# SumitTarafder/Figbird

Measured on AMD Instinct MI355X. Metric: gaps/sec (+ filled-bases/sec), synthetic 1e5-gap set recipe, jump-library fill pass, higher is better.
Workload: dtype f64

## Files before the change

### figbird_amd/api.py

```python
from __future__ import annotations

import ctypes as C
import os
from dataclasses import dataclass
from typing import List, Optional

import numpy as np

from . import build as _build

c_double_p = C.POINTER(C.c_double)
c_i32_p = C.POINTER(C.c_int32)
c_i64_p = C.POINTER(C.c_int64)
c_u8_p = C.POINTER(C.c_uint8)


class FigModel(C.Structure):
    _fields_ = [
        ("max_read_length", C.c_int32), ("error_pos_dist", c_double_p), ("in_pos_dist", c_double_p),
        ("del_pos_dist", c_double_p), ("error_type_probs", C.c_double * 25),
        ("insert_len_dist_smoothed", c_double_p), ("max_insert_size", C.c_int32),
        ("insert_threshold_min", C.c_int32), ("insert_threshold_max", C.c_int32), ("gap_prob_cutoff", C.c_int32),
        ("partial_flag", C.c_int32), ("unmapped_flag", C.c_int32), ("script_itr", C.c_int32),
        ("max_distance", C.c_int32), ("read_length", C.c_int32), ("neg_overlap", C.c_int32),
# ... 17 lines not shown
class FigGapResults(C.Structure):
    _fields_ = [
        ("filled_len", c_i32_p), ("gaptofill", c_i32_p), ("str_off", c_i64_p), ("str", C.c_char_p),
        ("str_capacity", C.c_int64),
        ("dbg_max_cand", C.c_int32), ("dbg_n_cand", c_i32_p), ("dbg_cand_i", c_i32_p), ("dbg_cand_lik", c_double_p),
        ("dbg_n_place", c_i32_p),
        ("draw_pos", c_i32_p), ("draw_isz", c_i32_p), ("draw_len", c_i32_p),
        ("dbg_plane_cols", C.c_int32), ("dbg_plane_reads", C.c_int32), ("dbg_counts", c_double_p), ("dbg_read_maxlv", c_double_p),
    ]


class FigStats(C.Structure):
    _fields_ = [("kernel_ms", C.c_double), ("h2d_ms", C.c_double), ("d2h_ms", C.c_double),
                ("packed_bytes", C.c_int64), ("place_calls", C.c_int64), ("alg_flops", C.c_double),
                ("n_launches", C.c_int32), ("pad0", C.c_int32), ("spec_flops", C.c_double),
                ("mle_alg_flops", C.c_double), ("mle_exec_flops", C.c_double)]


EXPORTS = ["fig_version", "fig_strerror", "fig_ctx_create", "fig_ctx_destroy", "fig_ctx_set_model",
           "fig_results_capacity", "fig_batch_upload", "fig_fill_resident", "fig_batch_free", "fig_fill_gaps",
           "fig_get_stats", "fig_batch_probe_reach", "fig_batch_set_ot_preset"]

_lib = None
_host = None


def load_library(path: Optional[str] = None) -> C.CDLL:
    global _lib
    if _lib is not None and path is None:
        return _lib
    p = path or _build.LIB
# ... 321 lines not shown
```

### figbird_amd/csrc/fig_abi.hip

```cpp
#include <hip/hip_runtime.h>

#include <algorithm>
#include <cstdio>
#include <cstdlib>
#include <cstring>
#include <new>
#include <vector>
#include <chrono>
#include <thread>
#include <mutex>

#include "../../include/figbird_hip.h"
#include "fig_engine.h"
#include "fig_pack.h"
#include "fig_abi_host.h"

#ifdef FIG_PROF
#define FIG_PROF_BEGIN() const unsigned long long _k0 = __builtin_readcyclecounter()
#define FIG_PROF_FLUSH() do { if (E.lane == 0) { atomicAdd(&B.counters[30], E.wait_cycles); atomicAdd(&B.counters[31], (unsigned long long)__builtin_readcyclecounter() - _k0); \
    for (int i = 0; i < 22; i++) if (E.prof[i]) atomicAdd(&B.counters[8 + i], E.prof[i]); \
    for (int i = 22; i < 40; i++) if (E.prof[i]) atomicAdd(&B.counters[32 + (i - 22)], E.prof[i]); } } while (0)
#else
#define FIG_PROF_BEGIN() ((void)0)
#define FIG_PROF_FLUSH() ((void)0)
// ... 194 lines not shown
    DevBuf d_model_tabs;
    fig_model hm;
    bool have_batch = false;
    FigDevBatch db;
    std::vector<FigDevGap> h_gaps;
    std::vector<int32_t> h_order;
    struct Cls { FigLaunchClass c; int blocks; int capacity; };
    std::vector<Cls> classes;
    std::vector<DevBuf> bufs;
    int64_t n_gaps = 0, n_ureads = 0, n_preads = 0, str_total = 0;
    std::vector<int64_t> h_str_off;
    int nslots = 32;
    std::vector<FigLane> lanes;
    fig_stats stats;
    int sh_on = FIG_SH_SC;
    std::vector<uint8_t> h_ot;
    uint8_t *d_ot = nullptr;
};

static int dev_alloc(fig_ctx *ctx, size_t bytes, void **out) {
    DevBuf b;
    if (bytes == 0) bytes = 8;
    hipError_t e = hipMalloc(&b.p, bytes);
    if (e != hipSuccess) { ctx->last_hip = (int)e; return FIG_ENOMEM; }
    b.n = bytes;
    ctx->bufs.push_back(b);
    *out = b.p;
    return FIG_OK;
}

// ... 22 lines not shown
    int n = 0;
    if (hipGetDeviceCount(&n) != hipSuccess || n <= 0) return FIG_ENODEV;
    if (device_ordinal < 0 || device_ordinal >= n) return FIG_ENODEV;
    if (hipSetDevice(device_ordinal) != hipSuccess) return FIG_ENODEV;
    hipDeviceProp_t prop;
    if (hipGetDeviceProperties(&prop, device_ordinal) != hipSuccess) return FIG_ENODEV;
    fig_ctx *ctx = new (std::nothrow) fig_ctx();
    if (!ctx) return FIG_ENOMEM;
    ctx->device = device_ordinal;
    ctx->n_cu = prop.multiProcessorCount > 0 ? prop.multiProcessorCount : 256;
    if (hipStreamCreate(&ctx->stream) != hipSuccess || hipEventCreate(&ctx->ev0) != hipSuccess || hipEventCreate(&ctx->ev1) != hipSuccess) {
        delete ctx;
        return FIG_EHIP;
    }
    memset(&ctx->stats, 0, sizeof(ctx->stats));
    ctx->sh_on = fig_knobs_from_env(0).sh_on;
    *out = ctx;
    return FIG_OK;
}

static void free_batch(fig_ctx *ctx) {
    for (auto &b : ctx->bufs) if (b.p) hipFree(b.p);
    ctx->bufs.clear();
    ctx->d_ot = nullptr;
    ctx->have_batch = false;
    ctx->classes.clear();
    for (auto &l : ctx->lanes) { if (l.stream) hipStreamDestroy(l.stream); if (l.done) hipEventDestroy(l.done); if (l.h_ctl) hipHostFree(l.h_ctl); if (l.h_items) hipHostFree(l.h_items); if (l.h_entries) hipHostFree(l.h_entries); }
    ctx->lanes.clear();
}

extern "C" void fig_batch_free(fig_ctx *ctx) {
// ... 60 lines not shown

static hipError_t launch_any(fig_ctx *ctx, const fig_ctx::Cls &c, const FigDevBatch &db, hipStream_t stream, FigKind kind, int blocks, const void *list, int n, int qsel = 0) {
    if (c.c.tiles > 0) return launch_kind<true, 512>(ctx, c, db, stream, kind, blocks, list, n, qsel);
    if (c.c.lds_tab) return c.c.nt == 256 ? launch_kind<true, 256>(ctx, c, db, stream, kind, blocks, list, n, qsel) : launch_kind<true, 512>(ctx, c, db, stream, kind, blocks, list, n, qsel);
    return launch_kind<false, 512>(ctx, c, db, stream, kind, blocks, list, n, qsel);
}

extern "C" int fig_batch_upload(fig_ctx *ctx, const fig_gap_batch *b) {
    if (!ctx || !b) return FIG_EINVAL;
    if (!ctx->have_model) return FIG_EINVAL;
    hipSetDevice(ctx->device);
    free_batch(ctx);
    const fig_model *m = &ctx->hm;
    hipEventRecord(ctx->ev0, ctx->stream);
    FigPacked K;
    int prc = fig_pack(m, b, sizeof(FigState), K);
    if (prc) return prc;
    int64_t ng = K.n_gaps;
    ctx->h_gaps = K.gaps; ctx->h_order = K.order; ctx->h_str_off = K.str_off;
    ctx->str_total = K.str_total; ctx->n_gaps = ng;
    ctx->n_ureads = (int64_t)K.u_pos.size(); ctx->n_preads = (int64_t)K.p_pos.size();
    ctx->classes.clear();
    const bool log = fig_knobs_from_env(0).log;
    for (const FigLaunchClass &lc : K.classes) {
        fig_ctx::Cls c;
        c.c = lc;
        int per_cu = (int)std::max<size_t>(1, std::min<size_t>((160 * 1024) / std::max<size_t>(lc.lds, 1), (size_t)(2048 / lc.nt)));
        per_cu = std::min(per_cu, 8);
        c.capacity = ctx->n_cu * per_cu;
        c.blocks = std::min<int>(lc.q_end - lc.q_begin, c.capacity);
// ... 265 lines not shown
    ctx->stats.d2h_ms = ms;
#ifdef FIG_PROF
    { const char *nm[14] = {"A.wait", "B.wait", "-", "M.finish", "PR.pre", "PR.estep", "PR.mid", "PR.mle", "PR.post", "A.chain", "A.logexp", "A.work", "B.work", "M.chains"};
      for (int i = 0; i < 14; i++) fprintf(stderr, "[figprof] %-9s %8.1f Gcycles = %5.1f %% of wave-cycles\n", nm[i], cnt[8 + i] / 1e9, cnt[31] ? 100.0 * cnt[8 + i] / cnt[31] : 0.0);
      { const char *mn[4] = {"M.setup", "M.hint", "M.rounds", "M.surv"};
        for (int i = 0; i < 4; i++) fprintf(stderr, "[figprof] %-9s %8.1f Gcycles = %5.1f %% of wave-cycles\n", mn[i], cnt[22 + i] / 1e9, cnt[31] ? 100.0 * cnt[22 + i] / cnt[31] : 0.0); }
      fprintf(stderr, "[figprof] raw slots:"); for (int i = 0; i < 22; i++) fprintf(stderr, " %d:%.1f", i, cnt[8 + i] / 1e9); for (int i = 22; i < 40; i++) fprintf(stderr, " %d:%.1f", i, cnt[32 + i - 22] / 1e9); fprintf(stderr, "\n");
      fprintf(stderr, "[figprof] barrier wait %.3f of %.3f wave-Gcycles = %.1f %%\n", cnt[30] / 1e9, cnt[31] / 1e9, cnt[31] ? 100.0 * cnt[30] / cnt[31] : 0.0); }
#endif
    if (knobs.log) fprintf(stderr, "[figsched] useful flops %.4g, speculative evaluations executed %.4g (%.1f %% discarded)\n", (double)cnt[1], (double)cnt[2], cnt[2] ? 100.0 * (1.0 - ((double)cnt[1] / (double)cnt[2])) : 0.0);
    ctx->stats.place_calls = (int64_t)cnt[0];
    ctx->stats.alg_flops = (double)cnt[1];
    ctx->stats.spec_flops = (double)cnt[2];
    ctx->stats.mle_alg_flops = (double)cnt[3];
    ctx->stats.mle_exec_flops = (double)cnt[4];
    return fig_compact_results(ng, hstr.data(), ctx->h_str_off.data(), out);
}

extern "C" int fig_fill_gaps(fig_ctx *ctx, const fig_gap_batch *batch, fig_gap_results *out) { return fig_fill_gaps_once(ctx, batch, out); }

extern "C" int fig_get_stats(const fig_ctx *ctx, fig_stats *out) {
    if (!ctx || !out) return FIG_EINVAL;
    *out = ctx->stats;
    return FIG_OK;
}
```

### figbird_amd/csrc/fig_abi_host.h

```cpp
#ifndef FIG_ABI_HOST_H
#define FIG_ABI_HOST_H
#include <algorithm>
#include <cmath>
#include <cstdlib>
#include <cstring>
#include <vector>
#include "../../include/figbird_hip.h"
#include "fig_types.h"
#include "fig_gaprules.h"

static inline const char *fig_strerror_text(int code) {
    switch (code) {
        case FIG_OK: return "ok";
        case FIG_EINVAL: return "invalid argument";
        case FIG_ENODEV: return "no usable HIP device (libfighip has no CPU path)";
        case FIG_ENOMEM: return "out of memory";
        case FIG_EHIP: return "HIP runtime error";
        case FIG_ENOSPC: return "result string buffer too small";
        case FIG_EUNSUP: return "input outside the supported envelope";
        default: return "unknown error";
    }
}

static inline int fig_model_check(const fig_model *m) {
// ... 89 lines not shown
static int fig_fill_gaps_once(fig_ctx *ctx, const fig_gap_batch *batch, fig_gap_results *out) {
    int rc = fig_batch_upload(ctx, batch);
    if (rc) return rc;
    rc = fig_fill_resident(ctx, out);
    fig_batch_free(ctx);
    return rc;
}

struct FigKnobs {
    bool seq;
    bool lanes_serial;
    bool log;
    int minc;
    double ipw;
    int sh_on;
};

static FigKnobs fig_knobs_from_env(int unmapped) {
    FigKnobs k;
    const char *sched = getenv("FIG_SCHED"), *ser = getenv("FIG_LANES"), *mc = getenv("FIG_MIN_CHUNK"), *ipw = getenv("FIG_ITEMS_PER_WG");
    const char *ev = getenv("FIG_ESTEP"), *sc = getenv("FIG_SH_CHUNKS");
    k.seq = sched && strcmp(sched, "seq") == 0;
    k.lanes_serial = ser && strcmp(ser, "serial") == 0;
    k.log = getenv("FIG_SCHED_LOG") != nullptr;
    k.minc = mc ? std::max(1, atoi(mc)) : 16;
    k.ipw = ipw ? std::max(1.0, atof(ipw)) : (unmapped ? 12.0 : 6.0);
    k.sh_on = (ev && !strcmp(ev, "pair")) ? 0 : (sc ? std::max(1, std::min(FIG_SH_SC, atoi(sc))) : FIG_SH_SC);
    return k;
}

struct FigRound { std::vector<int> items, entries; int chunk = 0, n_active = 0; };

static void fig_plan_round(const std::vector<int> &ids, const int32_t *ctl, int capacity, int nsplit, int slots_cap, int minc, double ipw_base,
                           int &n_active_max, FigRound &R) {
    std::vector<int> &items = R.items, &entries = R.entries;
    items.clear(); entries.clear();
    R.chunk = 0; R.n_active = 0;
    for (int g : ids) if (ctl[(size_t)g * 4] == 1) R.n_active++;
    if (R.n_active == 0) return;
    long long rem_total = 0;
    for (int g : ids) if (ctl[(size_t)g * 4] == 1) rem_total += std::max(0, ctl[(size_t)g * 4 + 2] - ctl[(size_t)g * 4 + 1]);
    n_active_max = std::max(n_active_max, R.n_active);
// ... 21 lines not shown
```

### figbird_amd/csrc/fig_engine.h

```cpp
#ifndef FIG_ENGINE_H
#define FIG_ENGINE_H

#include "fig_types.h"

#ifdef FIG_EMU
#include <cmath>
#include <cstring>
#define FIG_D static inline
#define FIG_NOINLINE
#define FIG_HD static inline
#define FIG_SYNC() ((void)0)
FIG_D double fig_log10(double x) { return log10(x); }
FIG_D double fig_log(double x) { return log(x); }
FIG_D double fig_exp(double x) { return exp(x); }
FIG_D double fig_pow10(double x) { return pow(10, x); }
FIG_D int fig_atomic_add_i32(int *p, int v) { int o = *p; *p += v; return o; }
FIG_D void fig_atomic_max_i32(int *p, int v) { if (v > *p) *p = v; }
FIG_D int fig_atomic_fetch_add_i32(int *p, int v) { int o = *p; *p += v; return o; }
FIG_D void fig_atomic_min_i32(int *p, int v) { if (v < *p) *p = v; }
FIG_D void fig_atomic_or_i32(int *p, int v) { *p |= v; }
FIG_D void fig_atomic_add_u64(unsigned long long *p, unsigned long long v) { *p += v; }
FIG_D unsigned long long fig_shfl_down_u64(unsigned long long v, int off) { (void)v; (void)off; return 0; }
#else
#include <hip/hip_runtime.h>
// ... 81 lines not shown
    unsigned char gap_left[32], gap_right[32];
    unsigned char partial_left[100], partial_right[100];
    double FP[6][5], FQ[6][5];
    double red_v[16]; int red_i[16];
    double bc_d; int bc_i, bc_j;
    int ibuf[8];
    double lik;
    int ctl[8];
    int tm_lo[16], tm_hi[16], tm_len[16], tm_tis0[16], tm_dir[16];
    int tm_aux[16]; long long tm_woff[16];
    double wv_v[32]; int wv_o[32];
    short sh_lo[FIG_SH_SC * FIG_SH_C], sh_hi[FIG_SH_SC * FIG_SH_C];
    int sh_tis0[FIG_SH_SC * FIG_SH_C];
    unsigned sh_woff[FIG_SH_SC * FIG_SH_C];
    unsigned char sh_len[FIG_SH_SC * FIG_SH_C], sh_aux[FIG_SH_SC * FIG_SH_C];
    unsigned sh_irr[16], sh_pad;
    int mle_next, pad_mn;
    int fin_i[8];
    FigLoop L;
    unsigned long long flops_useful; int n_place, pad_np;
    int dbg_j, pad_dj;
};

struct FigTrip { int v[3]; };



struct FigScr {
    double *cnt;
    double *ncnt;
    double *tmp;
    int *pc;
    int *nci;
    unsigned char *accf;
    unsigned char *mdone;
    int *cov;
// ... 454 lines not shown
```

### figbird_amd/csrc/fig_engine_core.h

```cpp

struct FigWin { int lo, hi; int tis0; int dir; };

FIG_D FigWin fig_window_unmapped(const FigEng &E, int pos1, int len, int G, int gapoffset) {
    const FigDevModel &M = *E.M;
    long long gsl = E.g->gapStart;
    FigWin w;
    int lo = -(len - 1), hi = G - 1;
    if ((long long)pos1 < gsl) {
        w.tis0 = (int)(gsl - pos1 + len); w.dir = 1;
        int a = M.Tmin - w.tis0, b = M.Tmax - w.tis0;
        if (a > lo) lo = a;
        if (b < hi) hi = b;
    } else {
        int p = pos1 + gapoffset;
        w.tis0 = (int)(p - gsl + len); w.dir = -1;
        int a = w.tis0 - M.Tmax, b = w.tis0 - M.Tmin;
        if (a > lo) lo = a;
        if (b < hi) hi = b;
    }
    w.lo = lo; w.hi = hi;
    return w;
}

FIG_D FigWin fig_window_partial(const FigEng &E, int pos1, int ref_pos, int len, int G, int gapoffset, int shift_always) {
// ... 288 lines not shown
                        if (S.gap_right[s4n + j] == rc) match++;
                    }
                    if (remn - match <= 2) return s4n;
                }
                part_count++;
                if (part_count > FIG_READ_CAP) break;
            }
        }
    }
    return 0;
}

FIG_D int fig_initialize(FigEng &E, int gl, int negGapCheck) {
    FigState &S = *E.S;
    int cg = E.capG;
    if (E.tid == 0) { S.G = gl; fig_ise(E); S.region_perct = 0; }
    FIG_SYNC();
    int G = S.G;
    for (int x = E.tid; x < cg; x += E.nt) {
        if (x < G) { E.scr.cnt[x] = 0; E.scr.cnt[cg + x] = 0; E.scr.cnt[2 * cg + x] = 0; E.scr.cnt[3 * cg + x] = 0; E.scr.cnt[4 * cg + x] = 1;
                     for (int j = 0; j < 5; j++) E.scr.ncnt[j * cg + x] = 0; }
        for (int j = 0; j < 5; j++) E.scr.tmp[j * cg + x] = 0;
        E.scr.cov[x] = 0;
    }
    int nml = E.g->nU > E.g->nP ? E.g->nU : E.g->nP;
    for (int r = E.tid; r < nml; r += E.nt) E.scr.maxlv[r] = 0;
    for (int r = E.tid; r < E.g->nU; r += E.nt) { E.scr.hint[r] = FIG_NOPOS; E.scr.hint_e[r] = FIG_NOPOS; }
    FIG_SYNC();
    if (E.tid == 0) {
        int gfp = 0;
        if (S.side_limit > 0 && negGapCheck == 0) gfp = fig_find_contig_match(E);
// ... 949 lines not shown
```

### figbird_amd/csrc/fig_engine_sched.h

```cpp
#ifndef FIG_ENGINE_SCHED_H
#define FIG_ENGINE_SCHED_H

template <bool LDS>
FIG_D void fig_gap_begin(FigEng &E) {
    FigState &S = *E.S;
    const FigDevModel &M = *E.M;
    const FigDevGap &g = *E.g;
    int G0 = g.G0, nU = g.nU;
    if (E.tid == 0) {
        S.left = M.D; S.right = M.D; S.side_limit = 30; S.end_pos_max = 0;
        S.valid_count = S.invalid_count = 0;
        S.partial_read_count = M.partial_flag == 1 ? g.nP : 0;
        S.region_perct = 0; S.region_perct_max = 0;
        S.partial_read_len = M.partial_len;
        S.rep_flag = 0; S.one_side_repeat_flag = 0; S.large_gap_flag = g.lgf; S.comp_count = 0;
        S.left_max = 0; S.right_min = 0; S.discont_or_not = 0;
        S.psr_temp[0] = S.psr_temp[1] = S.psr_final[0] = S.psr_final[1] = -1;
        S.umaxleftf = S.umaxrightf = S.ucoverf = 0;
        S.num_itr = 0; S.overlap_threshold = (E.B->ot_preset && E.B->ot_preset[g.gapNo]) ? 5 : 0; S.gaptofill = 0;
        S.gl_len = S.gr_len = S.pl_len = S.pr_len = 0;
        S.cons_len = 1; E.scr.cons[0] = 4;
        E.scr.used_read_arr[0] = 0;
        S.best_len = S.cur_len = S.prev_len = S.orig_len = 0;
        S.flops_useful = 0; S.n_place = 0; S.dbg_j = -1; S.pad_dj = 0;
        fig_flank_tables(E);
        if (E.B->dbg_n_cand) E.B->dbg_n_cand[g.gapNo] = 0;
        if (E.B->draw_len) { E.B->draw_len[(long long)g.gapNo * 2] = -1; E.B->draw_len[(long long)g.gapNo * 2 + 1] = -1; }
    }
    for (int r = E.tid; r < nU; r += E.nt) {
        E.scr.saved[r] = 0; E.scr.mark[r] = 0; E.scr.org[r * 2] = -200; E.scr.org[r * 2 + 1] = 0;
        E.scr.frp[r * 2] = -200; E.scr.frp[r * 2 + 1] = 0;
        if (E.B->draw_pos) E.B->draw_pos[g.uBase + r] = (int)0x80000000;
    }
    for (int p = E.tid; p < g.nP; p += E.nt) {
        E.scr.ppos_org[p * 3] = 0; E.scr.ppos_org[p * 3 + 1] = -200; E.scr.ppos_org[p * 3 + 2] = 0;
        if (E.B->draw_pos) E.B->draw_pos[E.B->n_ureads + g.pBase + p] = (int)0x80000000;
    }
    FIG_SYNC();
    if (E.tid == 0) {
// ... 273 lines not shown
FIG_D unsigned char *fig_slot_mark(const FigPersist &P, int s, int capGg) { return fig_slot_cons(P, s) + 2 * fig_align8(capGg + 8); }

FIG_D void fig_state_save(FigEng &E, const FigPersist &P) {
    FIG_SYNC();
    const int n = (int)(sizeof(FigState) / 4);
    const int *src = (const int *)E.S; int *dst = (int *)P.state;
    for (int i = E.tid; i < n; i += E.nt) dst[i] = src[i];
    FIG_SYNC();
}
FIG_D void fig_state_load(FigEng &E, const FigPersist &P) {
    FIG_SYNC();
    const int n = (int)(sizeof(FigState) / 4);
    int *dst = (int *)E.S; const int *src = (const int *)P.state;
    for (int i = E.tid; i < n; i += E.nt) dst[i] = src[i];
    FIG_SYNC();
}

enum { FIG_BIND_SEQ = 0, FIG_BIND_EVAL = 1, FIG_BIND_REPLAY = 2 };
FIG_D void fig_bind(FigEng &E, const FigScr &work, const FigPersist &P, int mode, int slot, int capGg) {
    E.scr = work;
    E.scr.best = P.best; E.scr.orig = P.orig; E.scr.saved = P.saved;
    E.scr.repeatflag = P.repeatflag; E.scr.used_read_arr = P.used_read_arr; E.scr.lrmd = P.lrmd;
    E.scr.org = P.org; E.scr.ppos_org = P.ppos_org;
    if (mode == FIG_BIND_SEQ) { E.scr.prev = P.prev; }
    else {
        E.scr.cons = fig_slot_cons(P, slot); E.scr.mark = fig_slot_mark(P, slot, capGg);
        if (mode == FIG_BIND_EVAL) { E.scr.org = P.org_spec; E.scr.ppos_org = P.ppos_spec; }
    }
}

// ... 82 lines not shown
```

### figbird_amd/csrc/fig_engine_shared.h

```cpp
#ifndef FIG_ENGINE_SHARED_H
#define FIG_ENGINE_SHARED_H
#ifndef FIG_EMU
#define FIG_FI __device__ static __forceinline__

FIG_D unsigned fig_wave_max_u32(unsigned v) {
#define FIG_DPP_UMAX(ctrl, rmask) do { const unsigned y_ = (unsigned)__builtin_amdgcn_update_dpp(0, (int)v, ctrl, rmask, 0xf, false); v = y_ > v ? y_ : v; } while (0)
    FIG_DPP_UMAX(0x111, 0xf); FIG_DPP_UMAX(0x112, 0xf); FIG_DPP_UMAX(0x114, 0xf); FIG_DPP_UMAX(0x118, 0xf);
    FIG_DPP_UMAX(0x142, 0xa); FIG_DPP_UMAX(0x143, 0xc);
#undef FIG_DPP_UMAX
    return (unsigned)__builtin_amdgcn_readlane((int)v, 63);
}


template <int N>
FIG_FI void fig_weights_n(const double (&x)[N], double (&w)[N]) {
    double m[N], a[N], b[N], r[N], s[N], z[N], q[N], s_lo[N], t[N], lm_lo[N], ed[N], p_hi[N], p_lo[N], r_hi[N], sum[N], err[N], tl[N];
    int e[N];
#pragma unroll
    for (int i = 0; i < N; i++) { m[i] = __builtin_amdgcn_frexp_mant(x[i]); e[i] = __builtin_amdgcn_frexp_exp(x[i]); }
#pragma unroll
    for (int i = 0; i < N; i++) { const bool lowhalf = m[i] < 0.70710678118654752440; m[i] = lowhalf ? m[i] + m[i] : m[i]; e[i] = lowhalf ? e[i] - 1 : e[i]; }
#pragma unroll
    for (int i = 0; i < N; i++) { a[i] = m[i] - 1.0; b[i] = m[i] + 1.0; }
#pragma unroll
// ... 80 lines not shown
    double f[8], m1[8], m2[8];
#pragma unroll
    for (int b = 0; b < 4; b++) { m1[b] = ac[b].p * kc[0]; m1[4 + b] = ac[b].p * kc[2]; }
#pragma unroll
    for (int b = 0; b < 4; b++) { m2[b] = kc[1] * ac[b].q; m2[4 + b] = kc[3] * ac[b].q; }
#pragma unroll
    for (int i = 0; i < 8; i++) f[i] = m1[i] + m2[i];
    const double one = 1.0;
    if (NS == 32) { fig_sh_mul16(&p[0], f, one, &wc[0]); fig_sh_mul16(&p[16], f, one, &wc[8]); }
    else if (NS == 16) fig_sh_mul16(&p[0], f, one, &wc[0]);
    else if (NS == 8) fig_sh_mul8(&p[0], f, one, &wc[0]);
    else fig_sh_mul4(&p[0], f, one, &wc[0]);
}

template <int NS>
FIG_FI void fig_sh_chain(double (&p)[FIG_SH_C], const FigPQ *colp, int ncolE, fig_cu32p st, fig_cdp ktf, fig_cdp ktr, int L) {
    uint32_t w0[NS / 2], w1[NS / 2];
    double k0[4], k1[4];
    FigPQ a0[4], a1[4];
#pragma unroll
    for (int k = 0; k < NS / 2; k++) w0[k] = st[k];
    k0[0] = ktf[0]; k0[1] = ktf[1]; k0[2] = ktr[0]; k0[3] = ktr[1];
#pragma unroll
    for (int b = 0; b < 4; b++) a0[b] = colp[b * ncolE];
    int j = 0;
#ifndef FIG_SH_UNROLL
#define FIG_SH_UNROLL 2
#endif
    for (; j + 2 * FIG_SH_UNROLL <= L; j += 2 * FIG_SH_UNROLL) {
#pragma unroll
        for (int u = 0; u < FIG_SH_UNROLL; u++) {
            fig_sh_step<NS>(p, w0, k0, a0, w1, k1, a1, colp, ncolE, st, ktf, ktr, j + 2 * u + 1);
            fig_sh_step<NS>(p, w1, k1, a1, w0, k0, a0, colp, ncolE, st, ktf, ktr, j + 2 * u + 2);
        }
    }
    for (; j + 2 <= L; j += 2) {
        fig_sh_step<NS>(p, w0, k0, a0, w1, k1, a1, colp, ncolE, st, ktf, ktr, j + 1);
        fig_sh_step<NS>(p, w1, k1, a1, w0, k0, a0, colp, ncolE, st, ktf, ktr, j + 2);
    }
    if (j < L) fig_sh_step<NS>(p, w0, k0, a0, w1, k1, a1, colp, ncolE, st, ktf, ktr, j + 1);
}

template <int NS>
FIG_FI void fig_sh_unit(const int s0, FigState &S, const FigHotU &U, const FigPQ *PQ, fig_cu32p stream, fig_gdp prow, const int pst, const int o, const bool vo, const int ocalc) {
    const fig_lsp SL = (fig_lsp)&S;
    double p[FIG_SH_C];
#pragma unroll
    for (int i = 0; i < NS; i++) {
        const int s = s0 + i;
        const int lo = fig_u(SL->sh_lo[s]), hi = fig_u(SL->sh_hi[s]), tis0 = fig_u(SL->sh_tis0[s]), dir = (fig_u(SL->sh_aux[s]) & 4) ? 1 : -1;
        p[i] = 1.0;
        if (ocalc >= lo && ocalc <= hi) p[i] = ((fig_gcdp)U.insd)[tis0 + dir * ocalc];
    }
    fig_sh_chain<NS>(p, PQ + (ocalc + U.xoff), U.ncolE, stream + ((s0 & (FIG_SH_C - 1)) >> 1), (fig_cdp)U.kt_fwd, (fig_cdp)U.kt_rev, U.L);
    if (vo) {
        fig_gdp dst = prow + (long long)s0 * pst + (o + U.L - 1);
#pragma unroll
        for (int i = 0; i < NS; i++) dst[(long long)i * pst] = p[i];
    }
}

template <int CPL>
FIG_NOINLINE FIG_D void fig_hot_estep_sh(FigEng &E, int gapoffset) {
    constexpr bool LDS = true;
    constexpr int NR = 4;
    constexpr int KP = 2;
    FigState &S = *E.S;
    const fig_lsp SL = (fig_lsp)E.S;
    const FigHotU U = fig_hot_uniforms(E);
    const int G = U.G, nU = U.nU, cg = U.cg;
    const long long ub = U.ub;
    const FigPQ *PQ = fig_pq_ptr<LDS>(E);
    double *W = fig_w_ptr<LDS>(E);
    const int Wcap = U.Wcap;
    const int wave = fig_u(E.wave), lane = E.lane, tid = E.tid, nw = U.nw;
    const fig_cu32p stream0 = (fig_cu32p)(fig_uptr(fig_uptr(E.B)->ustream) + fig_u64(fig_uptr(E.g)->streamOff));
    const long long wbase = nU > 0 ? fig_u64(U.u_woff[ub]) : 0;
    const fig_gdp prow = (fig_gdp)fig_uptr(E.scr.wg);
    const int pst = Wcap;
    double acc[CPL];
#pragma unroll
    for (int m = 0; m < CPL; m++) acc[m] = 0;
    const int pb_c = wave & 3, pb_x0 = (wave >> 2) * CPL * U.wsz + lane;
    unsigned long long fl_acc = 0;
    uint32_t *plb = (uint32_t *)(fig_lds + fig_u(E.off_plb));
    const int Wn = G + U.L - 1;
    const int nT = (Wn + 63) >> 6;
    int scn = fig_u(E.sh_on);
    scn = scn < 1 ? 1 : (scn > FIG_SH_SC ? FIG_SH_SC : scn);
    FIG_SYNC();
    FIG_T0(E);
    for (int c0 = 0; c0 < nU; c0 += scn * FIG_SH_C) {
        const int nrd = nU - c0 < scn * FIG_SH_C ? nU - c0 : scn * FIG_SH_C;
        const int nc = (nrd + FIG_SH_C - 1) / FIG_SH_C;
        if (tid < FIG_SH_SC * FIG_SH_C) {
            const int r = c0 + tid;
            int lo = 0, hi = -1, tis0 = 0, dir = 1; bool irr = false;
            int len = 0, aux = 0; long long woff = 0;
            if (tid < nrd) {
                len = U.u_len[ub + r]; aux = U.u_aux[ub + r]; woff = U.u_woff[ub + r];
                const FigWin w = fig_window_u(U, U.u_pos[ub + r], len, gapoffset);
                lo = w.lo; hi = w.hi; tis0 = w.tis0; dir = w.dir;
                irr = ((aux >> 1) & 1) != 0 || len != U.L;
            }
            SL->sh_lo[tid] = (short)lo; SL->sh_hi[tid] = (short)hi; SL->sh_tis0[tid] = tis0; SL->sh_len[tid] = (unsigned char)len;
            SL->sh_aux[tid] = (unsigned char)((aux & 3) | (dir > 0 ? 4 : 0)); SL->sh_woff[tid] = (unsigned)(woff - wbase);
            const unsigned long long im = fig_ballot(irr);
            if (lane == 0) { SL->sh_irr[2 * wave] = (unsigned)(im & 0xffffffffULL); SL->sh_irr[2 * wave + 1] = (unsigned)(im >> 32); }
        }
// ... 1 lines not shown
        uint32_t plv_next = 0;
        if (wave < NR && c0 + wave < nU) {
            const int len = fig_u(SL->sh_len[wave]);
            const int ndw = 2 + ((len + 3) >> 2) + 4;
            if (lane < ndw) plv_next = ((fig_gcu32p)U.packed)[wbase + fig_u((int)SL->sh_woff[wave]) + ((len + 15) >> 4) + ((len + 31) >> 5) + lane];
        }
        FIG_TICK(E, 34);
        {
            const int nit = nT * nc;
            const int nfull = nit / nw, mleft = nit - nfull * nw;
            const fig_cu32p stc = stream0 + (long long)(c0 / FIG_SH_C) * U.L * (FIG_SH_C / 2);
            for (int k = 0; k < nfull; k++) {
                const int it = k * nw + wave, ci = it / nT, tl = it - ci * nT;
                const int ob = -(U.L - 1) + 64 * tl, o = ob + lane;
                const bool vo = o <= G - 1;
                fig_sh_unit<32>(ci * FIG_SH_C, S, U, PQ, stc + (long long)ci * U.L * (FIG_SH_C / 2), prow, pst, o, vo, vo ? o : ob);
            }
            if (mleft > 0) {
                int fsplit = 1;
                while (fsplit * 2 * mleft <= nw && fsplit < 8) fsplit *= 2;
                if (wave < mleft * fsplit) {
                    const int nsl = FIG_SH_C / fsplit;
                    const int it = nfull * nw + wave / fsplit, ci = it / nT, tl = it - ci * nT;
                    const int s0 = ci * FIG_SH_C + (wave % fsplit) * nsl;
                    const int ob = -(U.L - 1) + 64 * tl, o = ob + lane;
                    const bool vo = o <= G - 1;
                    const fig_cu32p stp = stc + (long long)ci * U.L * (FIG_SH_C / 2);
                    if (fsplit == 1) fig_sh_unit<32>(s0, S, U, PQ, stp, prow, pst, o, vo, vo ? o : ob);
                    else if (fsplit == 2) fig_sh_unit<16>(s0, S, U, PQ, stp, prow, pst, o, vo, vo ? o : ob);
                    else if (fsplit == 4) fig_sh_unit<8>(s0, S, U, PQ, stp, prow, pst, o, vo, vo ? o : ob);
                    else fig_sh_unit<4>(s0, S, U, PQ, stp, prow, pst, o, vo, vo ? o : ob);
                }
            }
        }
        FIG_TICK(E, 35);
        FIG_SYNC();
        double pn[NR][KP];
#pragma unroll
        for (int t = 0; t < NR; t++)
#pragma unroll
            for (int k = 0; k < KP; k++) { const int i = tid + k * U.nt; pn[t][k] = (i < Wn && c0 + t < nU) ? prow[(long long)t * pst + i] : 0.0; }
        for (int q0 = 0; q0 < nrd; q0 += NR) {
            const unsigned irr = (unsigned)fig_u((int)SL->sh_irr[q0 >> 5]) >> (q0 & 31);
            int g_lo = 0, g_hi = -1;
            if (lane < NR && c0 + q0 + lane < nU) { g_lo = SL->sh_lo[q0 + lane]; g_hi = SL->sh_hi[q0 + lane]; }
            if (wave < NR) {
// ... 189 lines not shown
            FIG_TICK(E, 38);
            FIG_SYNC();
            FIG_TICK(E, 39);
        }
        if (tid < nrd) {
            const bool isirr = (SL->sh_irr[tid >> 5] >> (tid & 31)) & 1u;
            if (!isirr && E.scr.hint_e[c0 + tid] != FIG_NOPOS) E.scr.maxlv[c0 + tid] = fig_log10(E.scr.maxlv[c0 + tid]);
        }
    }
#pragma unroll
    for (int i = 0; i < CPL; i++) {
        const int x = pb_x0 + i * U.wsz;
        if (x < G) E.scr.cnt[pb_c * cg + x] = acc[i];
    }
    E.flops += fl_acc;
    FIG_SYNC();
}

FIG_D bool fig_sh_applies(const FigEng &E, int cpl) {
    if (!E.sh_on || E.tiles > 0 || !E.pq_lds || E.nteams < 4 || cpl > 8 || cpl < 1) return false;
    if (!E.B->ustream || E.M->L < 32) return false;
    const FigState &S = *E.S;
    if (S.left < E.xoff) return false;
    const int Wn = S.G + E.M->L - 1;
    return Wn <= 2 * E.nt && (E.nw == 4 || E.nw == 8) && (long long)FIG_SH_SC * FIG_SH_C * E.Wcap <= (long long)E.B->capW;
}

#endif
#endif
```

### figbird_amd/csrc/fig_pack.h

```cpp
#ifndef FIG_PACK_H
#define FIG_PACK_H
#include <algorithm>
#include <cstdlib>
#include <cstring>
#include <vector>
#include "../../include/figbird_hip.h"
#include "fig_types.h"
#include "fig_gaprules.h"

static inline int code_of(char c) {
    switch (c) { case 'A': return 0; case 'C': return 1; case 'G': return 2; case 'T': return 3; default: return 4; }
}

static void pack_read(const char *s, int len, std::vector<uint32_t> &out) {
    int nw2 = (len + 15) >> 4, nwm = (len + 31) >> 5, nwp = ((len + 3) >> 2) + 4;
    size_t base = out.size();
    out.resize(base + nw2 + nwm + 2 + nwp, 0u);
    int cnt[5] = {0, 0, 0, 0, 0};
    for (int j = 0; j < len; j++) {
        int c = code_of(s[j]);
        if (c < 4) out[base + (j >> 4)] |= (uint32_t)c << ((j & 15) * 2);
        else out[base + nw2 + (j >> 5)] |= 1u << (j & 31);
        cnt[c]++;
    }
// ... 27 lines not shown
                        int nsplit; };

struct FigPacked {
    std::vector<FigDevGap> gaps;
    std::vector<int32_t> order;
    std::vector<uint8_t> flank, qual;
    std::vector<uint32_t> packed;
    std::vector<int32_t> u_pos, u_aux, u_len, p_pos, p_aux, p_clip, p_ref, p_len;
    std::vector<int64_t> u_woff, p_woff, p_qoff, str_off;
    std::vector<FigLaunchClass> classes;
    std::vector<uint8_t> ot_preset;
    bool ot_given = false;
    int capR = 1, capP = 1, capC = 1, capG = 8, capW = 0, capE = 0;
    int64_t str_total = 0, n_gaps = 0, persist_total = 0, stream_total = 0;
    int nslots = 64;
    int64_t packed_bytes() const {
        return (int64_t)(packed.size() * 4 + flank.size() + gaps.size() * sizeof(FigDevGap) + qual.size() +
                         (u_pos.size() * 3 + p_pos.size() * 5) * 4 + (u_woff.size() + p_woff.size() + p_qoff.size()) * 8);
    }
};

static int fig_pack(const fig_model *m, const fig_gap_batch *b, size_t state_bytes, FigPacked &K) {
    int64_t ng = b->n_gaps;
    if (ng < 0) return FIG_EINVAL;
    if (ng > 0 && (!b->gap_contig || !b->gap_start || !b->gap_len || !b->contig_off || !b->contig_seq || !b->p_read_off)) return FIG_EINVAL;
    if (m->unmapped_flag && ng > 0 && !b->u_read_off) return FIG_EINVAL;
    if (ng > 0) {
        if (b->p_read_off[0] < 0 || (m->unmapped_flag && b->u_read_off[0] < 0)) return FIG_EINVAL;
        for (int64_t g = 0; g < ng; g++) {
            if (b->p_read_off[g + 1] < b->p_read_off[g]) return FIG_EINVAL;
// ... 102 lines not shown
    {
        long long off = 0;
        for (int64_t g = 0; g < ng; g++) {
            FigDevGap &d = K.gaps[g];
            d.capGg = (gmax[g] + 7) & ~7; d.rangeCap = gap_range(d.G0, d.gpf1, d.gpf2); d.nslots = K.nslots;
            d.persistOff = off;
            off += (fig_persist_layout(nullptr, d.capGg, d.nU, d.nP, d.rangeCap, d.nslots, state_bytes, nullptr) + 255) & ~255LL;
        }
        K.persist_total = off;
    }
    struct ClsDef { int capGl, nt; };
    const ClsDef defs[] = {{448, 256}, {1216, 512}, {1600, 512}, {1 << 30, 512}};
    K.order.clear(); K.classes.clear();
    const int L1 = m->max_read_length - 1;
    int prevcap = 0;
    for (const ClsDef &cd : defs) {
        std::vector<int32_t> ids;
        int mx = 8, mxa = 8;
        for (int64_t g = 0; g < ng; g++)
            if (gmax[g] > prevcap && gmax[g] <= cd.capGl) { ids.push_back((int32_t)g); mx = std::max(mx, gmax[g]); mxa = std::max(mxa, K.gaps[g].alloc_arg); }
        prevcap = cd.capGl;
        if (ids.empty()) continue;
        std::stable_sort(ids.begin(), ids.end(), [&](int32_t a, int32_t c) { return cost[a] > cost[c]; });
        FigLaunchClass c;
        c.capG = (mxa + 7) & ~7;
        c.capGl = (mx + 7) & ~7;
        c.ncolE = (c.capGl + 2 * L1 + 7) & ~7;
        c.Wcap = (c.capGl + m->max_read_length + 7) & ~7;
        c.nt = cd.nt;
        const size_t LDS_MAX = 160 * 1024 - 1024;
// ... 20 lines not shown
                const long long mle = FIG_TILED_MLE_DOUBLES(c.ncolE, c.nt / 64);
                if (mle <= c.tiled_max && fixed + sizeof(double) * (size_t)mle > c.lds) c.lds = fixed + sizeof(double) * (size_t)mle;
            }
        }
        { const char *ev = getenv("FIG_CLASS_LANES");
          const int want = ev ? std::max(1, std::min(8, atoi(ev))) : 2;
          c.nsplit = (int)ids.size() >= (FIG_SPLIT_MIN_GAPS / 2) * want ? want : 1; }
        for (int part = 0; part < c.nsplit; part++) {
            c.q_begin = (int)K.order.size();
            for (size_t k = (size_t)part; k < ids.size(); k += (size_t)c.nsplit) { const int32_t id = ids[k]; K.gaps[id].cls = (int)K.classes.size(); K.order.push_back(id); }
            c.q_end = (int)K.order.size();
            K.classes.push_back(c);
        }
        K.capE = std::max(K.capE, c.ncolE);
        K.capW = std::max(K.capW, (c.tiles ? 8 : c.nteams) * c.Wcap + 1024);
        if (m->unmapped_flag && c.lds_tab && !c.tiles && c.nteams >= 4) K.capW = std::max(K.capW, FIG_SH_SC * FIG_SH_C * c.Wcap + 1024);
    }
    return FIG_OK;
}

static int64_t fig_pack_results_capacity(const fig_model *m, const fig_gap_batch *b) {
    int64_t tot = 0;
    for (int64_t g = 0; g < b->n_gaps; g++) {
        int a, lgf; float f1, f2;
        gap_alloc(m, b->gap_len[g], &a, &f1, &f2, &lgf);
        tot += std::max(a, b->gap_len[g]) + 1;
    }
    return tot;
}
#endif
```

### figbird_amd/csrc/fig_types.h

```cpp
#ifndef FIG_TYPES_H
#define FIG_TYPES_H
#include <stdint.h>

#define FIG_MAX_READLEN 200
#define FIG_READ_CAP 3000
#define FIG_MAX_GAP 100000
#define FIG_FLANK 208
#define FIG_DBL_MAX 1.7976931348623157e308
#define FIG_SH_C 32
#define FIG_SH_SC 4
#define FIG_SH_ONE 16
#define FIG_MLE_FB 208
#define FIG_TILED_MLE_DOUBLES(ncolE, nw) (7LL * (ncolE) + (long long)(nw) * FIG_MLE_FB + ((ncolE) + 15) / 16 + 16 + 8)

struct FigDevModel {
    int32_t L;
    int32_t Tmin, Tmax, cutoff;
    int32_t partial_flag, unmapped, script_itr, D, read_length, neg_overlap, partial_len, unm_limit;
    int32_t max_insert;
    double T[25];
    const double *e;
    const double *ome;
    const double *ome1;
    const double *m3;
    const double *insd;
    const double *qtab;
// ... 52 lines not shown
```

### include/figbird_hip.h

```cpp
#ifndef FIGBIRD_HIP_H
#define FIGBIRD_HIP_H

#include <stdint.h>

#ifdef __cplusplus
extern "C" {
#endif

#define FIG_ABI_VERSION 1

#define FIG_OK 0
#define FIG_EINVAL (-1)
#define FIG_ENODEV (-2)
#define FIG_ENOMEM (-3)
#define FIG_EHIP (-4)
#define FIG_ENOSPC (-5)
#define FIG_EUNSUP (-6)

typedef struct fig_ctx fig_ctx;

typedef struct fig_model {
    int32_t max_read_length;
    const double *error_pos_dist;
    const double *in_pos_dist;
// ... 59 lines not shown
    double *dbg_counts;
    double *dbg_read_maxlv;
} fig_gap_results;

typedef struct fig_stats {
    double kernel_ms;
    double h2d_ms, d2h_ms;
    int64_t packed_bytes;
    int64_t place_calls;
    double alg_flops;
    int32_t n_launches;
    int32_t pad0;
    double spec_flops;
    double mle_alg_flops;
    double mle_exec_flops;
} fig_stats;

int fig_version(void);
const char *fig_strerror(int code);

int fig_ctx_create(int device_ordinal, fig_ctx **out);
void fig_ctx_destroy(fig_ctx *ctx);
int fig_ctx_set_model(fig_ctx *ctx, const fig_model *model);

int64_t fig_results_capacity(const fig_model *model, const fig_gap_batch *batch);

int fig_batch_upload(fig_ctx *ctx, const fig_gap_batch *batch);
int fig_fill_resident(fig_ctx *ctx, fig_gap_results *out);
void fig_batch_free(fig_ctx *ctx);
int fig_fill_gaps(fig_ctx *ctx, const fig_gap_batch *batch, fig_gap_results *out);
// ... 11 lines not shown
```

Before: 23.84.

## Cache shared-prefix likelihood chain partials across repeated unmapped-read evaluations

Splits the per-read shifted likelihood chain into a prefix and suffix part. On the first evaluation for a given gap, offset and generation, it stores the partial products at tile boundaries in extra global scratch. Later evaluations with the same state reload those partials and compute only the remaining suffix steps. This costs extra scratch memory (capW grows per eligible gap), global stores on the fill pass, and a generation counter to invalidate the cache when state is restored or reinitialised.

Result: slower. 21.52 (-9.7%).

```diff
diff --git a/figbird_amd/api.py b/figbird_amd/api.py
--- a/figbird_amd/api.py
+++ b/figbird_amd/api.py
@@ -55,7 +55,8 @@
     _fields_ = [("kernel_ms", C.c_double), ("h2d_ms", C.c_double), ("d2h_ms", C.c_double),
                 ("packed_bytes", C.c_int64), ("place_calls", C.c_int64), ("alg_flops", C.c_double),
                 ("n_launches", C.c_int32), ("pad0", C.c_int32), ("spec_flops", C.c_double),
-                ("mle_alg_flops", C.c_double), ("mle_exec_flops", C.c_double)]
+                ("mle_alg_flops", C.c_double), ("mle_exec_flops", C.c_double),
+                ("pfx_fills", C.c_int64), ("pfx_reuses", C.c_int64)]
 
 
 EXPORTS = ["fig_version", "fig_strerror", "fig_ctx_create", "fig_ctx_destroy", "fig_ctx_set_model",
diff --git a/figbird_amd/csrc/fig_abi.hip b/figbird_amd/csrc/fig_abi.hip
--- a/figbird_amd/csrc/fig_abi.hip
+++ b/figbird_amd/csrc/fig_abi.hip
@@ -232,6 +232,7 @@
     std::vector<FigLane> lanes;
     fig_stats stats;
     int sh_on = FIG_SH_SC;
+    bool pfx_on = true;
     std::vector<uint8_t> h_ot;
     uint8_t *d_ot = nullptr;
 };
@@ -284,7 +285,7 @@
         return FIG_EHIP;
     }
     memset(&ctx->stats, 0, sizeof(ctx->stats));
-    ctx->sh_on = fig_knobs_from_env(0).sh_on;
+    { const FigKnobs k = fig_knobs_from_env(0); ctx->sh_on = k.sh_on; ctx->pfx_on = k.pfx_on; }
     *out = ctx;
     return FIG_OK;
 }
@@ -375,6 +376,7 @@
     const fig_model *m = &ctx->hm;
     hipEventRecord(ctx->ev0, ctx->stream);
     FigPacked K;
+    K.pfx_on = ctx->pfx_on && ctx->sh_on;
     int prc = fig_pack(m, b, sizeof(FigState), K);
     if (prc) return prc;
     int64_t ng = K.n_gaps;
@@ -670,6 +672,8 @@
     ctx->stats.spec_flops = (double)cnt[2];
     ctx->stats.mle_alg_flops = (double)cnt[3];
     ctx->stats.mle_exec_flops = (double)cnt[4];
+    ctx->stats.pfx_fills = (int64_t)cnt[5];
+    ctx->stats.pfx_reuses = (int64_t)cnt[6];
     return fig_compact_results(ng, hstr.data(), ctx->h_str_off.data(), out);
 }
 
diff --git a/figbird_amd/csrc/fig_abi_host.h b/figbird_amd/csrc/fig_abi_host.h
--- a/figbird_amd/csrc/fig_abi_host.h
+++ b/figbird_amd/csrc/fig_abi_host.h
@@ -127,18 +127,20 @@
     int minc;
     double ipw;
     int sh_on;
+    bool pfx_on;
 };
 
 static FigKnobs fig_knobs_from_env(int unmapped) {
     FigKnobs k;
     const char *sched = getenv("FIG_SCHED"), *ser = getenv("FIG_LANES"), *mc = getenv("FIG_MIN_CHUNK"), *ipw = getenv("FIG_ITEMS_PER_WG");
-    const char *ev = getenv("FIG_ESTEP"), *sc = getenv("FIG_SH_CHUNKS");
+    const char *ev = getenv("FIG_ESTEP"), *sc = getenv("FIG_SH_CHUNKS"), *px = getenv("FIG_SH_PREFIX");
     k.seq = sched && strcmp(sched, "seq") == 0;
     k.lanes_serial = ser && strcmp(ser, "serial") == 0;
     k.log = getenv("FIG_SCHED_LOG") != nullptr;
     k.minc = mc ? std::max(1, atoi(mc)) : 16;
     k.ipw = ipw ? std::max(1.0, atof(ipw)) : (unmapped ? 12.0 : 6.0);
     k.sh_on = (ev && !strcmp(ev, "pair")) ? 0 : (sc ? std::max(1, std::min(FIG_SH_SC, atoi(sc))) : FIG_SH_SC);
+    k.pfx_on = !(px && !strcmp(px, "0"));
     return k;
 }
 
diff --git a/figbird_amd/csrc/fig_engine.h b/figbird_amd/csrc/fig_engine.h
--- a/figbird_amd/csrc/fig_engine.h
+++ b/figbird_amd/csrc/fig_engine.h
@@ -119,12 +119,13 @@
     int sh_tis0[FIG_SH_SC * FIG_SH_C];
     unsigned sh_woff[FIG_SH_SC * FIG_SH_C];
     unsigned char sh_len[FIG_SH_SC * FIG_SH_C], sh_aux[FIG_SH_SC * FIG_SH_C];
-    unsigned sh_irr[16], sh_pad;
-    int mle_next, pad_mn;
+    unsigned sh_irr[16];
+    int pfx_G;
+    int mle_next, pfx_off;
     int fin_i[8];
     FigLoop L;
-    unsigned long long flops_useful; int n_place, pad_np;
-    int dbg_j, pad_dj;
+    unsigned long long flops_useful; int n_place, pfx_gen;
+    int dbg_j, pfx_cur;
 };
 
 struct FigTrip { int v[3]; };
diff --git a/figbird_amd/csrc/fig_engine_core.h b/figbird_amd/csrc/fig_engine_core.h
--- a/figbird_amd/csrc/fig_engine_core.h
+++ b/figbird_amd/csrc/fig_engine_core.h
@@ -326,7 +326,7 @@
 FIG_D int fig_initialize(FigEng &E, int gl, int negGapCheck) {
     FigState &S = *E.S;
     int cg = E.capG;
-    if (E.tid == 0) { S.G = gl; fig_ise(E); S.region_perct = 0; }
+    if (E.tid == 0) { S.G = gl; fig_ise(E); S.region_perct = 0; S.pfx_cur++; }
     FIG_SYNC();
     int G = S.G;
     for (int x = E.tid; x < cg; x += E.nt) {
diff --git a/figbird_amd/csrc/fig_engine_sched.h b/figbird_amd/csrc/fig_engine_sched.h
--- a/figbird_amd/csrc/fig_engine_sched.h
+++ b/figbird_amd/csrc/fig_engine_sched.h
@@ -22,7 +22,8 @@
         S.cons_len = 1; E.scr.cons[0] = 4;
         E.scr.used_read_arr[0] = 0;
         S.best_len = S.cur_len = S.prev_len = S.orig_len = 0;
-        S.flops_useful = 0; S.n_place = 0; S.dbg_j = -1; S.pad_dj = 0;
+        S.flops_useful = 0; S.n_place = 0; S.dbg_j = -1;
+        S.pfx_G = -1; S.pfx_off = 0; S.pfx_gen = -1; S.pfx_cur = 0;
         fig_flank_tables(E);
         if (E.B->dbg_n_cand) E.B->dbg_n_cand[g.gapNo] = 0;
         if (E.B->draw_len) { E.B->draw_len[(long long)g.gapNo * 2] = -1; E.B->draw_len[(long long)g.gapNo * 2 + 1] = -1; }
@@ -326,6 +327,8 @@
     int *dst = (int *)E.S; const int *src = (const int *)P.state;
     for (int i = E.tid; i < n; i += E.nt) dst[i] = src[i];
     FIG_SYNC();
+    if (E.tid == 0) E.S->pfx_gen = -1;
+    FIG_SYNC();
 }
 
 enum { FIG_BIND_SEQ = 0, FIG_BIND_EVAL = 1, FIG_BIND_REPLAY = 2 };
diff --git a/figbird_amd/csrc/fig_engine_shared.h b/figbird_amd/csrc/fig_engine_shared.h
--- a/figbird_amd/csrc/fig_engine_shared.h
+++ b/figbird_amd/csrc/fig_engine_shared.h
@@ -118,7 +118,7 @@
 }
 
 template <int NS>
-FIG_FI void fig_sh_chain(double (&p)[FIG_SH_C], const FigPQ *colp, int ncolE, fig_cu32p st, fig_cdp ktf, fig_cdp ktr, int L) {
+FIG_FI void fig_sh_steps(double (&p)[FIG_SH_C], const FigPQ *colp, int ncolE, fig_cu32p st, fig_cdp ktf, fig_cdp ktr, int n) {
     uint32_t w0[NS / 2], w1[NS / 2];
     double k0[4], k1[4];
     FigPQ a0[4], a1[4];
@@ -131,32 +131,61 @@
 #ifndef FIG_SH_UNROLL
 #define FIG_SH_UNROLL 2
 #endif
-    for (; j + 2 * FIG_SH_UNROLL <= L; j += 2 * FIG_SH_UNROLL) {
+    for (; j + 2 * FIG_SH_UNROLL <= n; j += 2 * FIG_SH_UNROLL) {
 #pragma unroll
         for (int u = 0; u < FIG_SH_UNROLL; u++) {
             fig_sh_step<NS>(p, w0, k0, a0, w1, k1, a1, colp, ncolE, st, ktf, ktr, j + 2 * u + 1);
             fig_sh_step<NS>(p, w1, k1, a1, w0, k0, a0, colp, ncolE, st, ktf, ktr, j + 2 * u + 2);
         }
     }
-    for (; j + 2 <= L; j += 2) {
+    for (; j + 2 <= n; j += 2) {
         fig_sh_step<NS>(p, w0, k0, a0, w1, k1, a1, colp, ncolE, st, ktf, ktr, j + 1);
         fig_sh_step<NS>(p, w1, k1, a1, w0, k0, a0, colp, ncolE, st, ktf, ktr, j + 2);
     }
-    if (j < L) fig_sh_step<NS>(p, w0, k0, a0, w1, k1, a1, colp, ncolE, st, ktf, ktr, j + 1);
-}
-
+    if (j < n) fig_sh_step<NS>(p, w0, k0, a0, w1, k1, a1, colp, ncolE, st, ktf, ktr, j + 1);
+}
 template <int NS>
-FIG_FI void fig_sh_unit(const int s0, FigState &S, const FigHotU &U, const FigPQ *PQ, fig_cu32p stream, fig_gdp prow, const int pst, const int o, const bool vo, const int ocalc) {
+FIG_FI void fig_sh_chain(double (&p)[FIG_SH_C], const FigPQ *colp, int ncolE, fig_cu32p st, fig_cdp ktf, fig_cdp ktr, int ja, int jb) {
+    fig_sh_steps<NS>(p, colp + ja, ncolE, st + ja * (FIG_SH_C / 2), ktf + 2 * ja, ktr + 2 * ja, jb - ja);
+}
+
+struct FigPfx { fig_gdp base; int ntp, mode; };
+
+template <int NS>
+FIG_FI void fig_sh_unit(const int s0, FigState &S, const FigHotU &U, const FigPQ *PQ, fig_cu32p stream, fig_gdp prow, const int pst, const int o, const bool vo, const int ocalc,
+                        const FigPfx &pf, const int tl) {
     const fig_lsp SL = (fig_lsp)&S;
     double p[FIG_SH_C];
-#pragma unroll
-    for (int i = 0; i < NS; i++) {
-        const int s = s0 + i;
-        const int lo = fig_u(SL->sh_lo[s]), hi = fig_u(SL->sh_hi[s]), tis0 = fig_u(SL->sh_tis0[s]), dir = (fig_u(SL->sh_aux[s]) & 4) ? 1 : -1;
-        p[i] = 1.0;
-        if (ocalc >= lo && ocalc <= hi) p[i] = ((fig_gcdp)U.insd)[tis0 + dir * ocalc];
-    }
-    fig_sh_chain<NS>(p, PQ + (ocalc + U.xoff), U.ncolE, stream + ((s0 & (FIG_SH_C - 1)) >> 1), (fig_cdp)U.kt_fwd, (fig_cdp)U.kt_rev, U.L);
+    const int jp = fig_u((pf.mode != 0 && tl < pf.ntp) ? U.L - 64 * (tl + 1) : 0);
+    const bool reuse = jp > 0 && pf.mode == 2;
+    const long long pstr = 64LL * pf.ntp;
+    if (reuse) {
+        const fig_gcdp pc = pf.base + ((long long)s0 * pstr + (o + U.L - 1));
+#pragma unroll
+        for (int i = 0; i < NS; i++) p[i] = pc[(long long)i * pstr];
+    } else {
+#pragma unroll
+        for (int i = 0; i < NS; i++) {
+            const int s = s0 + i;
+            const int lo = fig_u(SL->sh_lo[s]), hi = fig_u(SL->sh_hi[s]), tis0 = fig_u(SL->sh_tis0[s]), dir = (fig_u(SL->sh_aux[s]) & 4) ? 1 : -1;
+            p[i] = 1.0;
+            if (ocalc >= lo && ocalc <= hi) p[i] = ((fig_gcdp)U.insd)[tis0 + dir * ocalc];
+        }
+    }
+    const FigPQ *colp = PQ + (ocalc + U.xoff);
+    const fig_cu32p st = stream + ((s0 & (FIG_SH_C - 1)) >> 1);
+    if (jp == 0) fig_sh_chain<NS>(p, colp, U.ncolE, st, (fig_cdp)U.kt_fwd, (fig_cdp)U.kt_rev, 0, U.L);
+    else {
+        int ja = reuse ? jp : 0, jb = reuse ? U.L : jp;
+        for (;;) {
+            fig_sh_chain<NS>(p, colp, U.ncolE, st, (fig_cdp)U.kt_fwd, (fig_cdp)U.kt_rev, ja, jb);
+            if (jb == U.L) break;
+            const fig_gdp pc = pf.base + ((long long)s0 * pstr + (o + U.L - 1));
+#pragma unroll
+            for (int i = 0; i < NS; i++) pc[(long long)i * pstr] = p[i];
+            ja = jb; jb = U.L;
+        }
+    }
     if (vo) {
         fig_gdp dst = prow + (long long)s0 * pst + (o + U.L - 1);
 #pragma unroll
@@ -182,6 +211,11 @@
     const long long wbase = nU > 0 ? fig_u64(U.u_woff[ub]) : 0;
     const fig_gdp prow = (fig_gdp)fig_uptr(E.scr.wg);
     const int pst = Wcap;
+    FigPfx pf; pf.ntp = FIG_PFX_TILES(U.L); pf.mode = 0;
+    const long long pfx_off = (long long)FIG_SH_SC * FIG_SH_C * Wcap + 1024;
+    if ((fig_u(fig_uptr(E.g)->pad) & FIG_PFX_GAP_BIT) && pfx_off + FIG_PFX_DOUBLES(nU, U.L) <= (long long)fig_u(fig_uptr(E.B)->capW))
+        pf.mode = (fig_u(SL->pfx_G) == G && fig_u(SL->pfx_off) == fig_u(gapoffset) && fig_u(SL->pfx_gen) == fig_u(SL->pfx_cur)) ? 2 : 1;
+    pf.base = prow + pfx_off;
     double acc[CPL];
 #pragma unroll
     for (int m = 0; m < CPL; m++) acc[m] = 0;
@@ -197,6 +231,7 @@
     for (int c0 = 0; c0 < nU; c0 += scn * FIG_SH_C) {
         const int nrd = nU - c0 < scn * FIG_SH_C ? nU - c0 : scn * FIG_SH_C;
         const int nc = (nrd + FIG_SH_C - 1) / FIG_SH_C;
+        FigPfx pfc = pf; pfc.base = pf.base + (long long)c0 * 64 * pf.ntp;
         if (tid < FIG_SH_SC * FIG_SH_C) {
             const int r = c0 + tid;
             int lo = 0, hi = -1, tis0 = 0, dir = 1; bool irr = false;
@@ -228,7 +263,7 @@
                 const int it = k * nw + wave, ci = it / nT, tl = it - ci * nT;
                 const int ob = -(U.L - 1) + 64 * tl, o = ob + lane;
                 const bool vo = o <= G - 1;
-                fig_sh_unit<32>(ci * FIG_SH_C, S, U, PQ, stc + (long long)ci * U.L * (FIG_SH_C / 2), prow, pst, o, vo, vo ? o : ob);
+                fig_sh_unit<32>(ci * FIG_SH_C, S, U, PQ, stc + (long long)ci * U.L * (FIG_SH_C / 2), prow, pst, o, vo, vo ? o : ob, pfc, tl);
             }
             if (mleft > 0) {
                 int fsplit = 1;
@@ -240,10 +275,10 @@
                     const int ob = -(U.L - 1) + 64 * tl, o = ob + lane;
                     const bool vo = o <= G - 1;
                     const fig_cu32p stp = stc + (long long)ci * U.L * (FIG_SH_C / 2);
-                    if (fsplit == 1) fig_sh_unit<32>(s0, S, U, PQ, stp, prow, pst, o, vo, vo ? o : ob);
-                    else if (fsplit == 2) fig_sh_unit<16>(s0, S, U, PQ, stp, prow, pst, o, vo, vo ? o : ob);
-                    else if (fsplit == 4) fig_sh_unit<8>(s0, S, U, PQ, stp, prow, pst, o, vo, vo ? o : ob);
-                    else fig_sh_unit<4>(s0, S, U, PQ, stp, prow, pst, o, vo, vo ? o : ob);
+                    if (fsplit == 1) fig_sh_unit<32>(s0, S, U, PQ, stp, prow, pst, o, vo, vo ? o : ob, pfc, tl);
+                    else if (fsplit == 2) fig_sh_unit<16>(s0, S, U, PQ, stp, prow, pst, o, vo, vo ? o : ob, pfc, tl);
+                    else if (fsplit == 4) fig_sh_unit<8>(s0, S, U, PQ, stp, prow, pst, o, vo, vo ? o : ob, pfc, tl);
+                    else fig_sh_unit<4>(s0, S, U, PQ, stp, prow, pst, o, vo, vo ? o : ob, pfc, tl);
                 }
             }
         }
@@ -463,6 +498,10 @@
         if (x < G) E.scr.cnt[pb_c * cg + x] = acc[i];
     }
     E.flops += fl_acc;
+    if (tid == 0 && pf.mode != 0) {
+        if (pf.mode == 1) { SL->pfx_G = G; SL->pfx_off = gapoffset; SL->pfx_gen = SL->pfx_cur; }
+        fig_atomic_add_u64(&E.B->counters[pf.mode == 1 ? 5 : 6], 1ULL);
+    }
     FIG_SYNC();
 }
 
diff --git a/figbird_amd/csrc/fig_pack.h b/figbird_amd/csrc/fig_pack.h
--- a/figbird_amd/csrc/fig_pack.h
+++ b/figbird_amd/csrc/fig_pack.h
@@ -65,6 +65,9 @@
     int capR = 1, capP = 1, capC = 1, capG = 8, capW = 0, capE = 0;
     int64_t str_total = 0, n_gaps = 0, persist_total = 0, stream_total = 0;
     int nslots = 64;
+    bool pfx_on = true;
+    int64_t pfx_cap = FIG_PFX_CAP;
+    int64_t pfx_doubles = 0;
     int64_t packed_bytes() const {
         return (int64_t)(packed.size() * 4 + flank.size() + gaps.size() * sizeof(FigDevGap) + qual.size() +
                          (u_pos.size() * 3 + p_pos.size() * 5) * 4 + (u_woff.size() + p_woff.size() + p_qoff.size()) * 8);
@@ -197,6 +200,7 @@
     K.order.clear(); K.classes.clear();
     const int L1 = m->max_read_length - 1;
     int prevcap = 0;
+    int capW0 = 0;
     for (const ClsDef &cd : defs) {
         std::vector<int32_t> ids;
         int mx = 8, mxa = 8;
@@ -247,8 +251,21 @@
         }
         K.capE = std::max(K.capE, c.ncolE);
         K.capW = std::max(K.capW, (c.tiles ? 8 : c.nteams) * c.Wcap + 1024);
-        if (m->unmapped_flag && c.lds_tab && !c.tiles && c.nteams >= 4) K.capW = std::max(K.capW, FIG_SH_SC * FIG_SH_C * c.Wcap + 1024);
-    }
+        capW0 = std::max(capW0, (c.tiles ? 8 : c.nteams) * c.Wcap + 1024);
+        if (m->unmapped_flag && c.lds_tab && !c.tiles && c.nteams >= 4) {
+            const int rows = FIG_SH_SC * FIG_SH_C * c.Wcap + 1024;
+            int64_t pfx = 0;
+            for (int32_t id : ids) {
+                const int64_t need = FIG_PFX_DOUBLES(K.gaps[id].nU, m->max_read_length);
+                if (!K.pfx_on || need > K.pfx_cap) continue;
+                K.gaps[id].pad |= FIG_PFX_GAP_BIT;
+                pfx = std::max(pfx, need);
+            }
+            capW0 = std::max(capW0, rows);
+            K.capW = std::max(K.capW, (int)(rows + pfx));
+        }
+    }
+    K.pfx_doubles = K.capW - capW0;
     return FIG_OK;
 }
 
diff --git a/figbird_amd/csrc/fig_types.h b/figbird_amd/csrc/fig_types.h
--- a/figbird_amd/csrc/fig_types.h
+++ b/figbird_amd/csrc/fig_types.h
@@ -10,6 +10,10 @@
 #define FIG_SH_C 32
 #define FIG_SH_SC 4
 #define FIG_SH_ONE 16
+#define FIG_PFX_TILES(L) (((L) - 1) / 64)
+#define FIG_PFX_DOUBLES(nU, L) ((long long)(((nU) + FIG_SH_C - 1) / FIG_SH_C * FIG_SH_C) * 64 * FIG_PFX_TILES(L))
+#define FIG_PFX_CAP (1 << 19)
+#define FIG_PFX_GAP_BIT 2
 #define FIG_MLE_FB 208
 #define FIG_TILED_MLE_DOUBLES(ncolE, nw) (7LL * (ncolE) + (long long)(nw) * FIG_MLE_FB + ((ncolE) + 15) / 16 + 16 + 8)
 
diff --git a/include/figbird_hip.h b/include/figbird_hip.h
--- a/include/figbird_hip.h
+++ b/include/figbird_hip.h
@@ -97,6 +97,8 @@
     double spec_flops;
     double mle_alg_flops;
     double mle_exec_flops;
+    int64_t pfx_fills;
+    int64_t pfx_reuses;
 } fig_stats;
 
 int fig_version(void);
```
